# Project-SEA-Stack/HydroChrono

Hardware: AMD Instinct MI355X
Metric: hydro-force evals/sec (all bodies) (higher is better)
Workload: dtype f64

## Files before the change

hydrochrono_amd/csrc/hc_kernels.hpp:

```cpp
#pragma once
#include <hip/hip_runtime.h>

#include <cstddef>

#include "hc_limits.hpp"
#include "hc_tail.hpp"

namespace hc {


struct Panel {
    const double* base;
    int ntiles;
    int ngp;
};
inline size_t panel_doubles(int ntiles, int ngp) { return static_cast<size_t>(ntiles) * ngp * 128; }

struct HistoryView {
    const double* state;
    int N, D;
    double t;
    const double* ring_t;
    const double* ring_v;
    const double* ring_vT;
// ... 245 lines not shown
ScatterLaunch scatter_launch_config(ScatterArgs& a);
FinalizeLaunch finalize_launch_config(FinalizeArgs& a);
struct StepLaunch {
    int nblocks = 0;
    size_t smem = 0;
    int MT = 0;
    static constexpr int U = 2;
};
StepLaunch step_launch_config(const StepArgs& a, int mt);
struct BlockLaunch {
    int nblocks = 0;
    size_t smem = 0;
    int MT = 0, R = 0, NB = 0, WPS = 0;
};
BlockLaunch block_launch_config(const BlockArgs& a, int mt, BlockArgs* with_lds_layout);

void launch_relayout_rirf(const double* d_Kb_6xDxS, double* d_K, int ngp, int D, int S, int row0, double scale, hipStream_t stream);
void launch_relayout_rowmajor(const double* d_src, int rows, int cols, double* d_panel, int ngp, int row0, hipStream_t stream);
void launch_conv_step(const StepArgs& a, int mt, hipStream_t stream);
void launch_conv_block(const BlockArgs& a, int mt, hipStream_t stream);
void launch_reduce_block(const ReduceArgs& r, hipStream_t stream);
int reduce_block_grid(const ReduceArgs& r);
void launch_finalize(const FinalizeArgs& a, hipStream_t stream);
void launch_near_split(const NearArgs& a, hipStream_t stream);
void launch_wide_step(const WideStepArgs& a, hipStream_t stream);
void launch_scatter(const ScatterArgs& a, hipStream_t stream);
void launch_taper(const TaperArgs& a, hipStream_t stream);
void launch_eta_synthesis(const double* d_t, int nt, const double* d_amp, const double* d_omega, const double* d_phase, int nf,
                          double ramp_duration, double* d_eta, hipStream_t stream);
void launch_added_mass_mv(const double* d_M, int rows, int cols, const double* d_w, double c, double* d_R, hipStream_t stream);
void launch_added_mass_mv_tagged(const double* d_M, int rows, int cols, const double* d_w, const double* d_R_in, double c,
                                 unsigned long long* d_tagged, unsigned long long seq, const double* d_canary_in, unsigned long long* d_canary_out,
                                 hipStream_t stream);
void launch_unrelayout(const Panel& K, int Dloc, int D, int S, double* d_out, hipStream_t stream);
void launch_extract_series(const Panel& K, int row, int col, int D, int S, double* d_out, hipStream_t stream);
void launch_ring_transpose(const double* d_ring_v, int Hcap, int HcapT, int D, double* d_ring_vT, hipStream_t stream);
void launch_synth_rirf(double* d_K, int ntiles, int ngp, int Dloc, int D, int S, int row0, double dt, unsigned long long seed, double rho,
                       hipStream_t stream);

struct TailKhatArgs {
    Panel K;
    const double* width;
    const double* tw;
    double* Khat;
    int Dloc, D, S, NP;
};

struct TailFwdArgs {
    const double* ring_vT;
    int HcapT, Hcap, head;
    int D, S, NP;
    const double* tw;
    double* Xw;
};

struct TailGemvArgs {
    const double* Khat;
    const double* Xw;
    const double* Yin;
    double* Yout;
    int Dloc, ncols;
    int bin_lo, bin_hi;
    int col_lo, col_hi;
    int x_shift;
    int rows_per_wg;
};

struct TailInvArgs {
    const double* Y;
    const double* tw;
    double* tail;
    int Dloc, Dpad;
};
constexpr int kTailGemvRows = 32;
int tail_gemv_lds_bytes(const TailGemvArgs& g);
int tail_gemv_grid(const TailGemvArgs& g);
hipError_t launch_tail_khat(const TailKhatArgs& a, int N, hipStream_t s);
hipError_t launch_tail_fwd(const TailFwdArgs& a, int N, hipStream_t s);
void launch_tail_gemv(const TailGemvArgs& a, hipStream_t s);
hipError_t launch_tail_inv(const TailInvArgs& a, int N, hipStream_t s);

}
```

hydrochrono_amd/csrc/hc_pass.cpp:

```cpp
#include "hc_internal.hpp"

using namespace hc::detail;

namespace hc {
namespace detail {

StepViews make_views(const hc_ctx* c) {
    StepViews v{};
    const bool irregular = c->wave_kind == hc::kWaveIrregular;
    v.kex.base   = c->d_kex.p;
    v.kex.ntiles = c->ntiles;
    v.kex.ngp    = c->ngp_ex;
    v.ex.L        = c->L;
    v.ex.ex_tau   = c->d_ex_tau.p;
    v.ex.ex_width = c->d_ex_width.p;
    v.ex.eta_t    = c->d_eta_t.p;
    v.ex.eta      = c->d_eta.p;
    v.ex.nt       = c->nt;
    v.ex.eta_dt   = irregular ? (c->eta_record ? c->eta_h : c->irr.simulation_dt) : 1.0;
    v.ex.eta_t0   = (irregular && !c->eta_t.empty()) ? c->eta_t.front() : 0.0;
    return v;
}


// ... 134 lines not shown
    c->spec.far_cur = c->spec.far_next = 0;
    if (k_changed)
        for (auto& f : c->spec_form) f.khat_ok = false;
}

namespace {

int spec_n_index(int N) { return N == 256 ? 0 : (N == 512 ? 1 : 2); }
int spec_form_index(const hc_ctx* c) { return c->radiation_tail == hc::kTailFormUniform ? 1 : 0; }

bool spec_eligible(const hc_ctx* c, bool direct) {
    const auto& pl = c->plan;
    if (c->radiation_tail != hc::kTailFormLevelled && c->radiation_tail != hc::kTailFormUniform) return false;
    hc::TailLevel lv[hc::kTailLevelsMax];
    const int nlev = hc::tail_levels(c->S, c->radiation_tail, lv);
    if (nlev < 1) return false;
    if (direct) {
        if (!c->dk_tail_gemv.ok()) return false;
        for (int l = 0; l < nlev; ++l)
            if (!c->dk_tail_fwd[spec_n_index(lv[l].N)].ok() || !c->dk_tail_inv[spec_n_index(lv[l].N)].ok()) return false;
    }
    if (c->conv_mode == 1 && !c->proc_ready) return false;
    if (c->pass_ahead == 1 || (c->pass_ahead == 2 && c->ahead_now && pass_ahead_size_ok(c))) return false;
    const int L = c->lookahead;
    const int NP = hc::tail_partitions(c->S);
    if ((L != 16 && L != 32) || c->D >= 1024 || NP < 1 || NP * c->D > hc::kTailMaxCols) return false;
    if (!pl.valid || pl.own_zero || pl.sub != 0) return false;
    const int head = hc::tail_head_lags(lv, nlev);
    for (int j = 0; j < L; ++j)
        if (pl.s_defer[j] >= 0 || pl.s_cut[j] >= head) return false;
    return hc::tail_grid_ok(c->times, c->tau, pl.dt, pl.tgrid[1]);
}

void spec_twiddles(hc_ctx* c, hc_ctx::SpectralLevel& lev) {
    const int N = lev.lv.N;
    if (lev.tw.n == static_cast<size_t>(2 * N)) return;
    std::vector<double> tw(2 * static_cast<size_t>(N));
    const double pi = 3.14159265358979323846;
    for (int k = 0; k < N; ++k) {
        const int q = (4 * k) / N, r = k - q * (N / 4);
        const double cr = std::cos(2.0 * pi * r / N), sr = std::sin(2.0 * pi * r / N);
        double co = cr, si = sr;
        if (q == 1) { co = -sr; si = cr; }
        if (q == 2) { co = -cr; si = -sr; }
        if (q == 3) { co = sr; si = -cr; }
        tw[2 * k]     = co;
        tw[2 * k + 1] = -si;
    }
    lev.tw.alloc(tw.size());
    HC_HIP(hipMemcpyAsync(lev.tw.p, tw.data(), tw.size() * sizeof(double), hipMemcpyHostToDevice, c->stream));
    HC_HIP(hipStreamSynchronize(c->stream));
}

void spec_dispatch_gemv(hc_ctx* c, const hc_ctx::SpectralLevel& lev, hipStream_t stream, bool direct, int bin_lo, int bin_hi, int col_lo, int col_hi, int x_shift,
                        const double* Yin, double* Yout) {
    if (bin_hi <= bin_lo || col_hi <= col_lo) return;
    hc::TailGemvArgs g{};
    g.Khat = lev.khat.p;
    g.Xw   = lev.xw.p;
    g.Yin  = Yin;
    g.Yout = Yout;
    g.Dloc = c->Dloc;
    g.ncols = lev.lv.NP * c->D;
    g.bin_lo = bin_lo;
    g.bin_hi = bin_hi;
    g.col_lo = col_lo;
    g.col_hi = col_hi;
    g.x_shift = x_shift;
    g.rows_per_wg = hc::kTailGemvRows;
    const double bytes = 16.0 * (bin_hi - bin_lo) * (static_cast<double>(c->Dloc) * (col_hi - col_lo) + (col_hi - col_lo) + (Yin ? 2.0 : 1.0) * c->Dloc);
    c->prof.tail_bytes += bytes;
    c->prof.tail_launches += 1;
    if (direct) {
        c->dq->dispatch(c->dk_tail_gemv, static_cast<uint32_t>(hc::tail_gemv_grid(g)), 256, static_cast<uint32_t>(hc::tail_gemv_lds_bytes(g)), &g, sizeof g,
                        direct_tag(c, hc::kEvTail));
        c->prof.direct_dispatches += 1;
        return;
    }
    hc::EventPair* ev = ev_begin(c, hc::kEvTail, stream);
    hc::launch_tail_gemv(g, stream);
    ev_end(ev, stream);
    c->prof.hip_launches += 1;
}

void spec_level_start(hc_ctx* c, hc_ctx::SpectralLevel& lev, bool top, hipStream_t stream, bool direct) {
    auto& sp = c->spec;
    const hc::TailLevel& lv = lev.lv;
    const int NP = lv.NP, D = c->D;
    const bool dd = direct;
    hc::TailFwdArgs f{};
    f.ring_vT = c->d_ring_vT.p;
    f.HcapT   = c->HcapT;
    f.Hcap    = c->Hcap;
    f.head    = c->head;
    f.D       = D;
    f.S       = c->S;
    f.NP      = NP;
    f.tw      = lev.tw.p;
    f.Xw      = lev.xw.p;
    c->prof.tail_bytes += 8.0 * NP * D * lv.N + 16.0 * lv.bins * NP * D;
    c->prof.tail_launches += 1;
    if (dd) {
        c->dq->dispatch(c->dk_tail_fwd[spec_n_index(lv.N)], static_cast<uint32_t>(NP * D), lv.N / 2, 0, &f, sizeof f, direct_tag(c, hc::kEvTail));
        c->prof.direct_dispatches += 1;
    } else {
        hc::EventPair* ev = ev_begin(c, hc::kEvTail, stream);
        HC_HIP(hc::launch_tail_fwd(f, lv.N, stream));
        ev_end(ev, stream);
        c->prof.hip_launches += 1;
    }
    double* Y = lev.y.p + static_cast<size_t>(top ? sp.cur : 0) * 2 * lv.bins * c->Dloc;
    if (NP > 1) {
        const int nch = hc::tail_far_chunks(sp.Q);
        if (!top || !hc::tail_level_far_ahead(lv) || sp.far_cur == 0) {
            spec_dispatch_gemv(c, lev, stream, dd, 0, lv.bins, D, NP * D, hc::tail_x_shift(false, D), nullptr, Y);
        } else {
            for (int k = 0; k < nch; ++k) {
                if (sp.far_cur & (1u << k)) continue;
                int lo, hi;
                hc::tail_level_chunk_bins(lv, k, nch, &lo, &hi);
                spec_dispatch_gemv(c, lev, stream, dd, lo, hi, D, NP * D, hc::tail_x_shift(false, D), nullptr, Y);
            }
        }
    }
    spec_dispatch_gemv(c, lev, stream, dd, 0, lv.bins, 0, D, 0, NP > 1 ? Y : nullptr, Y);
    hc::TailInvArgs iv{Y, lev.tw.p, lev.out.p, c->Dloc, c->Dpad};
    c->prof.tail_bytes += 16.0 * lv.bins * c->Dloc + 8.0 * lv.P * c->Dloc;
    c->prof.tail_launches += 1;
    if (dd) {
        c->dq->dispatch(c->dk_tail_inv[spec_n_index(lv.N)], static_cast<uint32_t>(c->Dloc), lv.N / 2, 0, &iv, sizeof iv, direct_tag(c, hc::kEvTail));
        c->prof.direct_dispatches += 1;
    } else {
        hc::EventPair* ev = ev_begin(c, hc::kEvTail, stream);
        HC_HIP(hc::launch_tail_inv(iv, lv.N, stream));
        ev_end(ev, stream);
        c->prof.hip_launches += 1;
    }
}

bool spec_ready(hc_ctx* c) {
    auto& form = c->spec_form[spec_form_index(c)];
    hc::TailLevel lv[hc::kTailLevelsMax];
    const int nlev = hc::tail_levels(c->S, c->radiation_tail, lv);
    if (nlev < 1) return false;
    if (form.nlev != nlev || form.S != c->S) form.khat_ok = false;
    form.nlev = nlev;
    form.S    = c->S;
    std::vector<hc::DeviceBuffer<double>*> fresh;
    auto grow = [&](hc::DeviceBuffer<double>& b, size_t n) {
        if (b.n >= n) return false;
        fresh.push_back(&b);
        b.alloc(n);
        return true;
    };
    try {
        for (int l = 0; l < nlev; ++l) {
            auto& lev = form.lev[l];
            lev.lv = lv[l];
            const size_t bins = static_cast<size_t>(lv[l].bins), ncols = static_cast<size_t>(lv[l].NP) * c->D;
            grow(lev.xw, 2 * bins * ncols);
            grow(lev.y, 4 * bins * c->Dloc);
            if (grow(lev.out, static_cast<size_t>(lv[l].P) * c->Dpad)) {
                HC_HIP(hipMemsetAsync(lev.out.p, 0, lev.out.n * sizeof(double), c->stream));
                HC_HIP(hipStreamSynchronize(c->stream));
            }
            if (grow(lev.khat, 2 * bins * c->Dloc * ncols)) form.khat_ok = false;
        }
    } catch (const Error&) {
        (void)hipGetLastError();
        for (auto* b : fresh) b->release();
        form.khat_ok      = false;
        c->radiation_tail = 0;
        return false;
    }
    for (int l = 0; l < nlev; ++l) spec_twiddles(c, form.lev[l]);
    if (!form.khat_ok) {
        for (int l = 0; l < nlev; ++l) spec_build_khat(c, form.lev[l]);
        form.khat_ok = true;
    }
    return form.khat_ok;
}

}

void launch_pass(hc_ctx* c, hipStream_t stream, bool with_exc, bool direct, bool spec_goes_on) {
    auto& sp = c->spec;
    const auto& pl = c->plan;
    const int L = c->lookahead;
    const int fi = spec_form_index(c);
    bool use_tail = false;
    if (spec_goes_on && sp.active && sp.form == fi && sp.k < sp.Q && std::fabs(pl.dt - sp.dt) <= 1e-9 * sp.dt) {
        const double tol = std::max(1e-9 * pl.dt, 64.0 * std::numeric_limits<double>::epsilon() * std::fabs(pl.tgrid[1]));
        use_tail = std::fabs(pl.tgrid[1] - (sp.t0 + sp.k * L * sp.dt)) <= tol;
    }
    if (!use_tail) {
        const bool follows = spec_goes_on && sp.active && sp.form == fi && sp.k == sp.Q &&
                             std::fabs(pl.tgrid[1] - (sp.t0 + sp.k * L * sp.dt)) <=
                                 std::max(1e-9 * pl.dt, 64.0 * std::numeric_limits<double>::epsilon() * std::fabs(pl.tgrid[1])) &&
                             std::fabs(pl.dt - sp.dt) <= 1e-9 * sp.dt;
        const unsigned far_made = follows ? sp.far_next : 0u;
        sp.active = false;
        if (spec_eligible(c, direct) && spec_ready(c)) {
            sp.form     = fi;
            sp.cur      = follows ? 1 - sp.cur : sp.cur;
            sp.far_cur  = far_made;
            sp.far_next = 0;
            sp.Q        = hc::tail_level_blocks(c->spec_form[fi].lev[0].lv, L);
            sp.k        = 0;
            sp.t0       = pl.tgrid[1];
            sp.dt       = pl.dt;
            sp.active   = true;
            use_tail = true;
        }
    }
    if (!use_tail) {
        const PassSetup ps = make_pass(c, with_exc, false);
        c->plan.has_exc    = ps.exc_block;
        issue_pass_chunks(c, ps, 0, ps.b.nchunks, true, stream, direct);
        issue_pass_reduce(c, ps, rows_P(c, false), rows_E(c, false), stream, direct);
        return;
    }
    auto& form = c->spec_form[fi];
    const int j0 = sp.k * L;
    TailRows rows;
    for (int l = 0; l < form.nlev; ++l) {
        auto& lev = form.lev[l];
        if (hc::tail_level_starts(lev.lv, j0)) spec_level_start(c, lev, l == 0, stream, direct);
        rows.tail[l] = lev.out.p;
        rows.j0[l]   = j0 % lev.lv.period;
    }
    const PassSetup ps = make_pass(c, with_exc, false, hc::tail_head_lags(&form.lev[form.nlev - 1].lv, 1));
    c->plan.has_exc    = ps.exc_block;
    issue_pass_chunks(c, ps, 0, ps.b.nchunks, true, stream, direct);
    issue_pass_reduce(c, ps, rows_P(c, false), rows_E(c, false), stream, direct, 0, &rows);
    const auto& top = form.lev[0];
    const int NP = top.lv.NP;
    if (hc::tail_level_far_ahead(top.lv) && sp.k >= 1) {
        const int ch = sp.k - 1, nch = hc::tail_far_chunks(sp.Q);
        int lo, hi;
        hc::tail_level_chunk_bins(top.lv, ch, nch, &lo, &hi);
        spec_dispatch_gemv(c, top, stream, direct, lo, hi, c->D, NP * c->D, hc::tail_x_shift(true, c->D), nullptr,
                           top.y.p + static_cast<size_t>(1 - sp.cur) * 2 * top.lv.bins * c->Dloc);
        sp.far_next |= 1u << ch;
    }
    sp.k += 1;
    sp.serial = c->plan_serial;
    c->prof.tail_blocks += 1;
}

void ahead_drop(hc_ctx* c) { c->ahead.active = false; }

void reset_schedule_state(hc_ctx* c) {
    c->gap_seen = c->gap_long = c->gap_long_lo = 0;
    c->gap_hint  = -1.0;
    c->ahead_now = hc::near_slices_for(c->D) > 1 && c->gap_threshold <= 0.0;
}

bool schedule_ahead_for_next_block(hc_ctx* c) {
    if (c->pass_ahead == 0 || c->lookahead > 32) return false;
    if (c->pass_ahead == 1) return true;
    if (!pass_ahead_size_ok(c)) return false;
    if (c->gap_seen >= std::max(4, c->lookahead / 4)) {
        c->ahead_now = 2 * (c->ahead_now ? c->gap_long_lo : c->gap_long) > c->gap_seen;
        c->gap_seen = c->gap_long = c->gap_long_lo = 0;
    }
    (c->ahead_now ? c->prof.schedule_blocks_ahead : c->prof.schedule_blocks_at_start) += 1;
    return c->ahead_now;
}

void ahead_issue_slice(hc_ctx* c, hipStream_t stream, bool direct) {
    auto& ah = c->ahead;
    if (!ah.active || ah.reduced) return;
    if (ah.Hcap != c->Hcap || ah.plan_serial != c->plan_serial) { ahead_drop(c); return; }
    const int pushed = ((c->head - ah.head0) % c->Hcap + c->Hcap) % c->Hcap;
    if (std::max(pushed, c->lookahead) + ah.Hv - 2 >= c->Hcap) { ahead_drop(c); return; }
    PassSetup ps;
    ps.b         = ah.args;
    ps.b.hist.ring_t  = c->d_ring_t.p;
    ps.b.hist.ring_v  = c->d_ring_v.p;
    ps.b.hist.ring_vT = c->d_ring_vT.p;
    ps.exc_block = ah.has_exc;
    ps.rad_once  = ah.rad_once;
// ... 213 lines not shown
```

hydrochrono_amd/csrc/hc_runtime.cpp:

```cpp
#include "hc_internal.hpp"

#include <sched.h>

#include <cctype>

#include <atomic>

using namespace hc::detail;

template <class T>
void hc::BarBuffer<T>::alloc(size_t count) {
    if (p) (void)hipFree(p);
    p       = nullptr;
    n       = 0;
    host_ok = false;
    if (count == 0) return;
    static const bool disabled = HC_TUNE_INT("HC_NO_BAR_STATE", 0) != 0;
    if (disabled) return;
    void* q = nullptr;
    if (hipExtMallocWithFlags(&q, count * sizeof(T), hipDeviceMallocFinegrained) != hipSuccess) {
        (void)hipGetLastError();
        return;
    }
    p = static_cast<T*>(q);
// ... 552 lines not shown
                *abandon      = true;
            }
            return false;
        }
        const unsigned long long bits = tag[0];
        double got;
        std::memcpy(&got, &bits, sizeof got);
        if (got != rv + cv * wv) {
            c->direct_why = "self-test of the direct dispatch: memory re-written through the PCIe BAR was read stale";
            (void)q->drain(2.0, lane);
            return false;
        }
    }
    if (!q->drain(2.0, lane)) {
        c->direct_why = "self-test of the direct dispatch timed out";
        *abandon      = true;
        return false;
    }
    return true;
}

#ifdef HC_TUNING
static const char* const kKernelObjectName = "/hc_kernels_tuning.co";
#else
static const char* const kKernelObjectName = "/hc_kernels.co";
#endif
__attribute__((constructor)) static void request_device_memory_queue_rings() {
    if (env_int("HC_QUEUE_DEV_MEM", 0) == 0) return;
    (void)setenv("HSA_ALLOCATE_QUEUE_DEV_MEM", "1", 0);
}

void setup_direct(hc_ctx* c) {
    c->direct_ready = false;
    if (env_int("HC_DIRECT", 1) == 0) { c->direct_why = "disabled by HC_DIRECT=0"; return; }
    if (!c->bar_state.host_ok || !c->bar_am.host_ok || !c->bar_selftest.host_ok) { c->direct_why = "the device's memory is not host-addressable"; return; }
    std::unique_ptr<hc::DirectQueue> q(new hc::DirectQueue);
    std::string why;
    if (!q->init(c->device, library_dir() + kKernelObjectName, &why)) { c->direct_why = why; return; }
    c->dk_finalize = q->find("finalize_kernelILi4ELb0EEEv");
    c->dk_finalize_slot = q->find("finalize_kernelILi4ELb1EEEv");
    c->dk_scatter  = q->find("scatter_kernelE");
    c->dk_near     = q->find("near_split_kernelE");
    c->dk_wide     = q->find("wide_step_kernelE");
    if (c->dk_wide.kernarg != sizeof(hc::WideStepArgs) || c->dk_wide.priv != 0) c->dk_wide = hc::DirectKernel{};
    if (c->dk_finalize_slot.kernarg != sizeof(hc::FinalizeArgs) || c->dk_finalize_slot.priv != 0) c->dk_finalize_slot = hc::DirectKernel{};
    c->slot_state = HC_TUNE_INT("HC_SLOT_STATE", 1) != 0 && c->dk_finalize_slot.ok() && c->N <= hc::kSlotStateMaxBodies;
    c->dk_step_hot[0] = q->find("step_hot_kernelILi1EEEv");
    c->dk_step_hot[1] = q->find("step_hot_kernelILi2EEEv");
    for (auto& k : c->dk_step_hot)
        if (k.kernarg != sizeof(hc::StepHotArgs) || k.priv != 0) k = hc::DirectKernel{};
    c->step_hot = c->slot_state && c->dk_step_hot[0].ok() && c->dk_step_hot[1].ok() && HC_TUNE_INT("HC_STEP_HOT", 1) != 0;
    c->step_halves = HC_TUNE_INT("HC_STEP_HALVES", 1) == 2 ? 2 : 1;
    c->dk_reduce   = q->find("reduce_block_kernelE");
    c->dk_tail_gemv = q->find("tail_gemvENS_12TailGemvArgsE");
    bool tail_ok    = c->dk_tail_gemv.kernarg == sizeof(hc::TailGemvArgs) && !c->dk_tail_gemv.priv;
    for (int i = 0; i < 3; ++i) {
        char frag[64];
        std::snprintf(frag, sizeof frag, "tail_fft_fwdILi%dEEEvNS_11TailFwdArgsE", 256 << i);
        c->dk_tail_fwd[i] = q->find(frag);
        std::snprintf(frag, sizeof frag, "tail_fft_invILi%dEEEvNS_11TailInvArgsE", 256 << i);
        c->dk_tail_inv[i] = q->find(frag);
        tail_ok = tail_ok && c->dk_tail_fwd[i].kernarg == sizeof(hc::TailFwdArgs) && c->dk_tail_inv[i].kernarg == sizeof(hc::TailInvArgs) && !c->dk_tail_fwd[i].priv &&
                  !c->dk_tail_inv[i].priv;
    }
    if (!tail_ok) {
        c->dk_tail_gemv = hc::DirectKernel{};
        for (int i = 0; i < 3; ++i) c->dk_tail_fwd[i] = c->dk_tail_inv[i] = hc::DirectKernel{};
    }
    c->dk_added_mass = q->find("added_mass_mv_tagged_kernelE");
    {
        hc::StepArgs a{};
        a.ngroups = 1;
        const hc::StepLaunch l = hc::step_launch_config(a, c->mt);
        char frag[64];
        std::snprintf(frag, sizeof frag, "conv_step_kernelILi%dELi%dEEEv", l.MT, hc::StepLaunch::U);
        c->dk_step = q->find(frag);
        if (c->dk_step.kernarg != sizeof(hc::StepArgs) || c->dk_step.priv != 0) c->dk_step = hc::DirectKernel{};
    }
    for (int depth : {16, 32}) {
        hc::BlockArgs a{}, b{};
        a.depth = depth;
        a.ngroups = 1;
        const hc::BlockLaunch l = hc::block_launch_config(a, c->mt_block, &b);
        char frag[96];
        std::snprintf(frag, sizeof frag, "conv_block_kernelILi%dELi%dELi%dELi%dEEEv", l.MT, l.R, l.NB, l.WPS);
        (depth == 16 ? c->dk_block16 : c->dk_block32) = q->find(frag);
        const hc::BlockLaunch lm = hc::block_launch_config(a, c->mt_mini, &b);
        std::snprintf(frag, sizeof frag, "conv_block_kernelILi%dELi%dELi%dELi%dEEEv", lm.MT, lm.R, lm.NB, lm.WPS);
        (depth == 16 ? c->dk_mini16 : c->dk_mini32) = q->find(frag);
        if (depth == 16) {
            const hc::BlockLaunch ln = hc::block_launch_config(a, c->mt_narrow, &b);
            std::snprintf(frag, sizeof frag, "conv_block_kernelILi%dELi%dELi%dELi%dEEEv", ln.MT, ln.R, ln.NB, ln.WPS);
            c->dk_narrow = q->find(frag);
        }
    }
#ifdef HC_TUNING
    {
        hc::BlockArgs a{}, b{};
        a.depth   = 64;
        a.ngroups = 1;
        const hc::BlockLaunch l = hc::block_launch_config(a, hc::kBlock64MT, &b);
        char frag[96];
        std::snprintf(frag, sizeof frag, "conv_block_kernelILi%dELi%dELi%dELi%dEEEv", l.MT, l.R, l.NB, l.WPS);
        c->dk_block64 = q->find(frag);
        if (c->dk_block64.kernarg != sizeof(hc::BlockArgs) || c->dk_block64.priv != 0) c->dk_block64 = hc::DirectKernel{};
    }
#endif
    if (!c->dk_narrow.ok() || c->dk_narrow.priv || c->dk_narrow.kernarg != sizeof(hc::BlockArgs)) {
        c->direct_why = "the narrow short-pass variant of the pass kernel is missing from hc_kernels.co";
        return;
    }
    if (!c->dk_mini16.ok() || !c->dk_mini32.ok() || c->dk_mini16.priv || c->dk_mini32.priv || c->dk_mini16.kernarg != sizeof(hc::BlockArgs) ||
        c->dk_mini32.kernarg != sizeof(hc::BlockArgs)) {
        c->direct_why = "the short-pass variant of the pass kernel is missing from hc_kernels.co";
        return;
// ... 63 lines not shown
```

hydrochrono_amd/csrc/hc_tail_kernels.hpp:

```cpp
#pragma once

namespace hc {

template <int N>
__device__ __forceinline__ void tail_fft_lds(double* __restrict__ re, double* __restrict__ im, const double* __restrict__ tw, bool inverse) {
    const int t = threadIdx.x;
    __syncthreads();
#pragma unroll 1
    for (int len = 2; len <= N; len <<= 1) {
        const int half = len >> 1;
        const int pos  = t & (half - 1);
        const int i    = (t - pos) * 2 + pos;
        const int j    = i + half;
        const int k    = pos * (N / len);
        const double wr = tw[2 * k], wi = inverse ? -tw[2 * k + 1] : tw[2 * k + 1];
        const double br = re[j], bi = im[j];
        const double pr = wr * br - wi * bi, pi = wr * bi + wi * br;
        const double ar = re[i], ai = im[i];
        re[i] = ar + pr;
        im[i] = ai + pi;
        re[j] = ar - pr;
        im[j] = ai - pi;
        __syncthreads();
    }
}

constexpr int tail_log2(int n) { return n <= 1 ? 0 : 1 + tail_log2(n >> 1); }
template <int N>
__device__ __forceinline__ int tail_bitrev(int k) {
    static_assert(N >= 4 && (N & (N - 1)) == 0, "a transform of 2^b points");
    return static_cast<int>(__brev(static_cast<unsigned>(k)) >> (32 - tail_log2(N)));
}


template <int N>
__global__ void __launch_bounds__(N / 2) tail_khat_kernel(TailKhatArgs a) {
    constexpr int P = N / 2, kBins = P + 1, kThreads = N / 2;
    __shared__ double re[N], im[N];
    const int t   = threadIdx.x;
    const int col = blockIdx.x % a.D;
    const int rp  = blockIdx.x / a.D;
    const int p   = rp % a.NP + 1;
    const int row = rp / a.NP;
    for (int k = t; k < N; k += kThreads) {
        const int s = p * P + k;
        double g = 0.0;
        if (k < P && s < a.S) g = a.width[s] * a.K.base[panel_offset(a.K.ngp, row, s * a.D + col)];
        const int kr = tail_bitrev<N>(k);
        re[kr] = g;
        im[kr] = 0.0;
    }
    tail_fft_lds<N>(re, im, a.tw, false);
    const size_t ncols = static_cast<size_t>(a.NP) * a.D;
    const size_t c     = static_cast<size_t>(p - 1) * a.D + col;
    for (int b = t; b < kBins; b += kThreads) {
        double* dst = a.Khat + 2 * ((static_cast<size_t>(b) * a.Dloc + row) * ncols + c);
        dst[0] = re[b];
        dst[1] = im[b];
    }
}


template <int N>
__global__ void __launch_bounds__(N / 2) tail_fft_fwd(TailFwdArgs a) {
    constexpr int P = N / 2, kBins = P + 1, kThreads = N / 2;
    __shared__ double re[N], im[N];
    const int t   = threadIdx.x;
    const int col = blockIdx.x % a.D;
    const int w   = blockIdx.x / a.D + 1;
    const double* __restrict__ series = a.ring_vT + static_cast<size_t>(col) * a.HcapT;
    for (int k = t; k < N; k += kThreads) {
        const int back = (w + 1) * P - 1 - k;
        double x = 0.0;
        if (k >= 1 && back <= a.S - 2) {
            int slot = (a.head - back) % a.Hcap;
            if (slot < 0) slot += a.Hcap;
            x = series[slot];
        }
        const int kr = tail_bitrev<N>(k);
        re[kr] = x;
        im[kr] = 0.0;
    }
    tail_fft_lds<N>(re, im, a.tw, false);
    const size_t ncols = static_cast<size_t>(a.NP) * a.D;
    const size_t c     = static_cast<size_t>(w - 1) * a.D + col;
    for (int b = t; b < kBins; b += kThreads) {
        double* dst = a.Xw + 2 * (static_cast<size_t>(b) * ncols + c);
        dst[0] = re[b];
        dst[1] = im[b];
    }
}

static constexpr int kTailGemvUnroll = 6;
static constexpr int kTailGemvBatch  = 4;

__global__ void __launch_bounds__(256) tail_gemv(TailGemvArgs a) {
    extern __shared__ double xs[];
    const int nbin_rows = (a.Dloc + a.rows_per_wg - 1) / a.rows_per_wg;
    const int bin       = a.bin_lo + blockIdx.x / nbin_rows;
    const int row0      = (blockIdx.x % nbin_rows) * a.rows_per_wg;
    const int n         = a.col_hi - a.col_lo;
    const double* __restrict__ xsrc = a.Xw + 2 * (static_cast<size_t>(bin) * a.ncols + a.col_lo + a.x_shift);
    for (int i = threadIdx.x; i < 2 * n; i += 256) xs[i] = xsrc[i];
    __syncthreads();
    const int lane = threadIdx.x & 63, wave = threadIdx.x >> 6;
    const int row_end = min(a.Dloc, row0 + a.rows_per_wg);
    const dvec2* __restrict__ kbin = reinterpret_cast<const dvec2*>(a.Khat + 2 * (static_cast<size_t>(bin) * a.Dloc * a.ncols + a.col_lo));
    for (int rb = row0 + wave * kTailGemvBatch; rb < row_end; rb += 4 * kTailGemvBatch) {
        double sr[kTailGemvBatch], si[kTailGemvBatch];
#pragma unroll
        for (int q = 0; q < kTailGemvBatch; ++q) sr[q] = si[q] = 0.0;
        for (int c0 = 0; c0 < n; c0 += 64 * kTailGemvUnroll) {
            dvec2 kv[kTailGemvBatch][kTailGemvUnroll];
#pragma unroll
            for (int q = 0; q < kTailGemvBatch; ++q) {
                const int row = min(rb + q, row_end - 1);
#pragma unroll
                for (int u = 0; u < kTailGemvUnroll; ++u) {
                    const int c = c0 + 64 * u + lane;
                    kv[q][u] = c < n ? __builtin_nontemporal_load(kbin + static_cast<size_t>(row) * a.ncols + c) : dvec2{0.0, 0.0};
                }
            }
#pragma unroll
            for (int u = 0; u < kTailGemvUnroll; ++u) {
                const int c = c0 + 64 * u + lane;
                const double xr = c < n ? xs[2 * c] : 0.0, xi = c < n ? xs[2 * c + 1] : 0.0;
#pragma unroll
                for (int q = 0; q < kTailGemvBatch; ++q) {
                    sr[q] = fma(kv[q][u].x, xr, sr[q]);
                    sr[q] = fma(-kv[q][u].y, xi, sr[q]);
                    si[q] = fma(kv[q][u].x, xi, si[q]);
                    si[q] = fma(kv[q][u].y, xr, si[q]);
                }
            }
        }
#pragma unroll
        for (int off = 32; off >= 1; off >>= 1) {
#pragma unroll
            for (int q = 0; q < kTailGemvBatch; ++q) {
                sr[q] += __shfl_xor(sr[q], off, 64);
                si[q] += __shfl_xor(si[q], off, 64);
            }
        }
        if (lane < kTailGemvBatch && rb + lane < row_end) {
            double yr = sr[0], yi = si[0];
#pragma unroll
            for (int q = 1; q < kTailGemvBatch; ++q)
                if (lane == q) {
                    yr = sr[q];
                    yi = si[q];
                }
            const size_t o = 2 * (static_cast<size_t>(bin) * a.Dloc + rb + lane);
            if (a.Yin) {
                yr = a.Yin[o] + yr;
                yi = a.Yin[o + 1] + yi;
            }
            a.Yout[o]     = yr;
            a.Yout[o + 1] = yi;
        }
    }
}

template <int N>
__global__ void __launch_bounds__(N / 2) tail_fft_inv(TailInvArgs a) {
    constexpr int P = N / 2, kThreads = N / 2;
    __shared__ double re[N], im[N];
    const int t   = threadIdx.x;
    const int row = blockIdx.x;
    for (int k = t; k < N; k += kThreads) {
        const int b = k <= P ? k : N - k;
        const double* y = a.Y + 2 * (static_cast<size_t>(b) * a.Dloc + row);
        const double yr = y[0];
        double yi       = (b == 0 || b == P) ? 0.0 : y[1];
        if (k > P) yi = -yi;
        const int kr = tail_bitrev<N>(k);
        re[kr] = yr;
        im[kr] = yi;
    }
    tail_fft_lds<N>(re, im, a.tw, true);
    for (int j = t; j < P; j += kThreads) a.tail[static_cast<size_t>(j) * a.Dpad + row] = re[P + j] * (1.0 / N);
}

int tail_gemv_lds_bytes(const TailGemvArgs& g) { return 16 * (g.col_hi - g.col_lo); }
int tail_gemv_grid(const TailGemvArgs& g) { return (g.bin_hi - g.bin_lo) * ((g.Dloc + g.rows_per_wg - 1) / g.rows_per_wg); }

template __global__ void tail_khat_kernel<256>(TailKhatArgs);
template __global__ void tail_khat_kernel<512>(TailKhatArgs);
template __global__ void tail_khat_kernel<1024>(TailKhatArgs);
template __global__ void tail_fft_fwd<256>(TailFwdArgs);
template __global__ void tail_fft_fwd<512>(TailFwdArgs);
template __global__ void tail_fft_fwd<1024>(TailFwdArgs);
template __global__ void tail_fft_inv<256>(TailInvArgs);
template __global__ void tail_fft_inv<512>(TailInvArgs);
template __global__ void tail_fft_inv<1024>(TailInvArgs);

#define HC_TAIL_BY_N(n, call)                                 \
    switch (n) {                                              \
        case 256: { constexpr int kN = 256; call; break; }    \
        case 512: { constexpr int kN = 512; call; break; }    \
        case 1024: { constexpr int kN = 1024; call; break; }  \
        default: return hipErrorInvalidValue;                 \
    }                                                         \
    return hipSuccess;

hipError_t launch_tail_khat(const TailKhatArgs& a, int N, hipStream_t s) {
    HC_TAIL_BY_N(N, hipLaunchKernelGGL(tail_khat_kernel<kN>, dim3(static_cast<unsigned>(a.Dloc) * a.NP * a.D), dim3(kN / 2), 0, s, a))
}
hipError_t launch_tail_fwd(const TailFwdArgs& a, int N, hipStream_t s) {
    HC_TAIL_BY_N(N, hipLaunchKernelGGL(tail_fft_fwd<kN>, dim3(static_cast<unsigned>(a.NP) * a.D), dim3(kN / 2), 0, s, a))
}
void launch_tail_gemv(const TailGemvArgs& a, hipStream_t s) {
    hipLaunchKernelGGL(tail_gemv, dim3(static_cast<unsigned>(tail_gemv_grid(a))), dim3(256), static_cast<unsigned>(tail_gemv_lds_bytes(a)), s, a);
}
hipError_t launch_tail_inv(const TailInvArgs& a, int N, hipStream_t s) {
    HC_TAIL_BY_N(N, hipLaunchKernelGGL(tail_fft_inv<kN>, dim3(static_cast<unsigned>(a.Dloc)), dim3(kN / 2), 0, s, a))
}
#undef HC_TAIL_BY_N

}
```

Before: 83070.

## Batch spectral tail levels that start together into grouped FFT/GEMV launches

```diff
diff --git a/hydrochrono_amd/csrc/hc_kernels.hpp b/hydrochrono_amd/csrc/hc_kernels.hpp
--- a/hydrochrono_amd/csrc/hc_kernels.hpp
+++ b/hydrochrono_amd/csrc/hc_kernels.hpp
@@ -321,6 +321,7 @@
     int D, S, NP;
     const double* tw;
     double* Xw;
+    int N;
 };
 
 struct TailGemvArgs {
@@ -340,13 +341,26 @@
     const double* tw;
     double* tail;
     int Dloc, Dpad;
-};
+    int N;
+};
+
+template <class Args>
+struct TailGroup {
+    Args lev[kTailLevelsMax];
+    int wg_end[kTailLevelsMax];
+};
+using TailFwdGroup  = TailGroup<TailFwdArgs>;
+using TailGemvGroup = TailGroup<TailGemvArgs>;
+using TailInvGroup  = TailGroup<TailInvArgs>;
+
 constexpr int kTailGemvRows = 32;
 int tail_gemv_lds_bytes(const TailGemvArgs& g);
 int tail_gemv_grid(const TailGemvArgs& g);
+inline int tail_fwd_grid(const TailFwdArgs& a) { return a.NP * a.D; }
+inline int tail_inv_grid(const TailInvArgs& a) { return a.Dloc; }
 hipError_t launch_tail_khat(const TailKhatArgs& a, int N, hipStream_t s);
-hipError_t launch_tail_fwd(const TailFwdArgs& a, int N, hipStream_t s);
-void launch_tail_gemv(const TailGemvArgs& a, hipStream_t s);
-hipError_t launch_tail_inv(const TailInvArgs& a, int N, hipStream_t s);
+hipError_t launch_tail_fwd(const TailFwdGroup& g, int workgroups, hipStream_t s);
+void launch_tail_gemv(const TailGemvGroup& g, int workgroups, int lds_bytes, hipStream_t s);
+hipError_t launch_tail_inv(const TailInvGroup& g, int workgroups, hipStream_t s);
 
 }
diff --git a/hydrochrono_amd/csrc/hc_pass.cpp b/hydrochrono_amd/csrc/hc_pass.cpp
--- a/hydrochrono_amd/csrc/hc_pass.cpp
+++ b/hydrochrono_amd/csrc/hc_pass.cpp
@@ -210,9 +210,8 @@
     HC_HIP(hipStreamSynchronize(c->stream));
 }
 
-void spec_dispatch_gemv(hc_ctx* c, const hc_ctx::SpectralLevel& lev, hipStream_t stream, bool direct, int bin_lo, int bin_hi, int col_lo, int col_hi, int x_shift,
-                        const double* Yin, double* Yout) {
-    if (bin_hi <= bin_lo || col_hi <= col_lo) return;
+hc::TailGemvArgs spec_gemv_args(const hc_ctx* c, const hc_ctx::SpectralLevel& lev, int bin_lo, int bin_hi, int col_lo, int col_hi, int x_shift, const double* Yin,
+                                double* Yout) {
     hc::TailGemvArgs g{};
     g.Khat = lev.khat.p;
     g.Xw   = lev.xw.p;
@@ -226,71 +225,112 @@
     g.col_hi = col_hi;
     g.x_shift = x_shift;
     g.rows_per_wg = hc::kTailGemvRows;
-    const double bytes = 16.0 * (bin_hi - bin_lo) * (static_cast<double>(c->Dloc) * (col_hi - col_lo) + (col_hi - col_lo) + (Yin ? 2.0 : 1.0) * c->Dloc);
-    c->prof.tail_bytes += bytes;
+    return g;
+}
+
+template <class Args, class GridOf>
+int spec_group_ends(hc::TailGroup<Args>& g, int n, GridOf grid_of) {
+    int end = 0;
+    for (int l = 0; l < hc::kTailLevelsMax; ++l) {
+        if (l < n) end += grid_of(g.lev[l]);
+        else g.lev[l] = g.lev[n - 1];
+        g.wg_end[l] = end;
+    }
+    return end;
+}
+
+void spec_dispatch_gemv(hc_ctx* c, hc::TailGemvGroup& g, int n, hipStream_t stream, bool direct) {
+    int lds = 0;
+    for (int l = 0; l < n; ++l) {
+        const hc::TailGemvArgs& a = g.lev[l];
+        lds = std::max(lds, hc::tail_gemv_lds_bytes(a));
+        c->prof.tail_bytes += 16.0 * (a.bin_hi - a.bin_lo) *
+                              (static_cast<double>(c->Dloc) * (a.col_hi - a.col_lo) + (a.col_hi - a.col_lo) + (a.Yin ? 2.0 : 1.0) * c->Dloc);
+    }
+    const int wgs = spec_group_ends(g, n, [](const hc::TailGemvArgs& a) { return hc::tail_gemv_grid(a); });
     c->prof.tail_launches += 1;
     if (direct) {
-        c->dq->dispatch(c->dk_tail_gemv, static_cast<uint32_t>(hc::tail_gemv_grid(g)), 256, static_cast<uint32_t>(hc::tail_gemv_lds_bytes(g)), &g, sizeof g,
-                        direct_tag(c, hc::kEvTail));
+        c->dq->dispatch(c->dk_tail_gemv, static_cast<uint32_t>(wgs), 256, static_cast<uint32_t>(lds), &g, sizeof g, direct_tag(c, hc::kEvTail));
         c->prof.direct_dispatches += 1;
         return;
     }
     hc::EventPair* ev = ev_begin(c, hc::kEvTail, stream);
-    hc::launch_tail_gemv(g, stream);
+    hc::launch_tail_gemv(g, wgs, lds, stream);
     ev_end(ev, stream);
     c->prof.hip_launches += 1;
 }
 
-void spec_level_start(hc_ctx* c, hc_ctx::SpectralLevel& lev, bool top, hipStream_t stream, bool direct) {
+void spec_dispatch_gemv(hc_ctx* c, const hc_ctx::SpectralLevel& lev, hipStream_t stream, bool direct, int bin_lo, int bin_hi, int col_lo, int col_hi, int x_shift,
+                        const double* Yin, double* Yout) {
+    if (bin_hi <= bin_lo || col_hi <= col_lo) return;
+    hc::TailGemvGroup g{};
+    g.lev[0] = spec_gemv_args(c, lev, bin_lo, bin_hi, col_lo, col_hi, x_shift, Yin, Yout);
+    spec_dispatch_gemv(c, g, 1, stream, direct);
+}
+
+void spec_levels_start(hc_ctx* c, hc_ctx::SpectralLevel* const* lev, int n, bool top, hipStream_t stream, bool direct) {
     auto& sp = c->spec;
-    const hc::TailLevel& lv = lev.lv;
-    const int NP = lv.NP, D = c->D;
-    const bool dd = direct;
-    hc::TailFwdArgs f{};
-    f.ring_vT = c->d_ring_vT.p;
-    f.HcapT   = c->HcapT;
-    f.Hcap    = c->Hcap;
-    f.head    = c->head;
-    f.D       = D;
-    f.S       = c->S;
-    f.NP      = NP;
-    f.tw      = lev.tw.p;
-    f.Xw      = lev.xw.p;
-    c->prof.tail_bytes += 8.0 * NP * D * lv.N + 16.0 * lv.bins * NP * D;
+    const int D = c->D;
+    hc::TailFwdGroup fg{};
+    hc::TailGemvGroup ng{};
+    hc::TailInvGroup ig{};
+    double* Y[hc::kTailLevelsMax];
+    for (int l = 0; l < n; ++l) {
+        const hc::TailLevel& lv = lev[l]->lv;
+        hc::TailFwdArgs& f = fg.lev[l];
+        f.ring_vT = c->d_ring_vT.p;
+        f.HcapT   = c->HcapT;
+        f.Hcap    = c->Hcap;
+        f.head    = c->head;
+        f.D       = D;
+        f.S       = c->S;
+        f.NP      = lv.NP;
+        f.tw      = lev[l]->tw.p;
+        f.Xw      = lev[l]->xw.p;
+        f.N       = lv.N;
+        c->prof.tail_bytes += 8.0 * lv.NP * D * lv.N + 16.0 * lv.bins * lv.NP * D;
+        Y[l] = lev[l]->y.p + static_cast<size_t>(top && l == 0 ? sp.cur : 0) * 2 * lv.bins * c->Dloc;
+    }
+    const int fwd_wgs = spec_group_ends(fg, n, [](const hc::TailFwdArgs& a) { return hc::tail_fwd_grid(a); });
     c->prof.tail_launches += 1;
-    if (dd) {
-        c->dq->dispatch(c->dk_tail_fwd[spec_n_index(lv.N)], static_cast<uint32_t>(NP * D), lv.N / 2, 0, &f, sizeof f, direct_tag(c, hc::kEvTail));
+    if (direct) {
+        c->dq->dispatch(c->dk_tail_fwd[spec_n_index(fg.lev[0].N)], static_cast<uint32_t>(fwd_wgs), fg.lev[0].N / 2, 0, &fg, sizeof fg, direct_tag(c, hc::kEvTail));
         c->prof.direct_dispatches += 1;
     } else {
         hc::EventPair* ev = ev_begin(c, hc::kEvTail, stream);
-        HC_HIP(hc::launch_tail_fwd(f, lv.N, stream));
+        HC_HIP(hc::launch_tail_fwd(fg, fwd_wgs, stream));
         ev_end(ev, stream);
         c->prof.hip_launches += 1;
     }
-    double* Y = lev.y.p + static_cast<size_t>(top ? sp.cur : 0) * 2 * lv.bins * c->Dloc;
-    if (NP > 1) {
-        const int nch = hc::tail_far_chunks(sp.Q);
-        if (!top || !hc::tail_level_far_ahead(lv) || sp.far_cur == 0) {
-            spec_dispatch_gemv(c, lev, stream, dd, 0, lv.bins, D, NP * D, hc::tail_x_shift(false, D), nullptr, Y);
-        } else {
-            for (int k = 0; k < nch; ++k) {
-                if (sp.far_cur & (1u << k)) continue;
-                int lo, hi;
-                hc::tail_level_chunk_bins(lv, k, nch, &lo, &hi);
-                spec_dispatch_gemv(c, lev, stream, dd, lo, hi, D, NP * D, hc::tail_x_shift(false, D), nullptr, Y);
+    for (int l = 0; l < n; ++l) {
+        const hc::TailLevel& lv = lev[l]->lv;
+        const int NP = lv.NP;
+        if (NP > 1) {
+            const int nch = hc::tail_far_chunks(sp.Q);
+            if (!(top && l == 0) || !hc::tail_level_far_ahead(lv) || sp.far_cur == 0) {
+                spec_dispatch_gemv(c, *lev[l], stream, direct, 0, lv.bins, D, NP * D, hc::tail_x_shift(false, D), nullptr, Y[l]);
+            } else {
+                for (int k = 0; k < nch; ++k) {
+                    if (sp.far_cur & (1u << k)) continue;
+                    int lo, hi;
+                    hc::tail_level_chunk_bins(lv, k, nch, &lo, &hi);
+                    spec_dispatch_gemv(c, *lev[l], stream, direct, lo, hi, D, NP * D, hc::tail_x_shift(false, D), nullptr, Y[l]);
+                }
             }
         }
-    }
-    spec_dispatch_gemv(c, lev, stream, dd, 0, lv.bins, 0, D, 0, NP > 1 ? Y : nullptr, Y);
-    hc::TailInvArgs iv{Y, lev.tw.p, lev.out.p, c->Dloc, c->Dpad};
-    c->prof.tail_bytes += 16.0 * lv.bins * c->Dloc + 8.0 * lv.P * c->Dloc;
+        ng.lev[l] = spec_gemv_args(c, *lev[l], 0, lv.bins, 0, D, 0, NP > 1 ? Y[l] : nullptr, Y[l]);
+        ig.lev[l] = hc::TailInvArgs{Y[l], lev[l]->tw.p, lev[l]->out.p, c->Dloc, c->Dpad, lv.N};
+        c->prof.tail_bytes += 16.0 * lv.bins * c->Dloc + 8.0 * lv.P * c->Dloc;
+    }
+    spec_dispatch_gemv(c, ng, n, stream, direct);
+    const int inv_wgs = spec_group_ends(ig, n, [](const hc::TailInvArgs& a) { return hc::tail_inv_grid(a); });
     c->prof.tail_launches += 1;
-    if (dd) {
-        c->dq->dispatch(c->dk_tail_inv[spec_n_index(lv.N)], static_cast<uint32_t>(c->Dloc), lv.N / 2, 0, &iv, sizeof iv, direct_tag(c, hc::kEvTail));
+    if (direct) {
+        c->dq->dispatch(c->dk_tail_inv[spec_n_index(ig.lev[0].N)], static_cast<uint32_t>(inv_wgs), ig.lev[0].N / 2, 0, &ig, sizeof ig, direct_tag(c, hc::kEvTail));
         c->prof.direct_dispatches += 1;
     } else {
         hc::EventPair* ev = ev_begin(c, hc::kEvTail, stream);
-        HC_HIP(hc::launch_tail_inv(iv, lv.N, stream));
+        HC_HIP(hc::launch_tail_inv(ig, inv_wgs, stream));
         ev_end(ev, stream);
         c->prof.hip_launches += 1;
     }
@@ -381,11 +421,18 @@
     auto& form = c->spec_form[fi];
     const int j0 = sp.k * L;
     TailRows rows;
+    hc_ctx::SpectralLevel* starting[hc::kTailLevelsMax];
+    int nstart = 0;
     for (int l = 0; l < form.nlev; ++l) {
         auto& lev = form.lev[l];
-        if (hc::tail_level_starts(lev.lv, j0)) spec_level_start(c, lev, l == 0, stream, direct);
+        if (hc::tail_level_starts(lev.lv, j0)) starting[nstart++] = &lev;
         rows.tail[l] = lev.out.p;
         rows.j0[l]   = j0 % lev.lv.period;
+    }
+    if (HC_TUNE_INT("HC_TAIL_GROUP", 1) != 0) {
+        if (nstart > 0) spec_levels_start(c, starting, nstart, j0 == 0, stream, direct);
+    } else {
+        for (int i = 0; i < nstart; ++i) spec_levels_start(c, starting + i, 1, j0 == 0 && i == 0, stream, direct);
     }
     const PassSetup ps = make_pass(c, with_exc, false, hc::tail_head_lags(&form.lev[form.nlev - 1].lv, 1));
     c->plan.has_exc    = ps.exc_block;
diff --git a/hydrochrono_amd/csrc/hc_runtime.cpp b/hydrochrono_amd/csrc/hc_runtime.cpp
--- a/hydrochrono_amd/csrc/hc_runtime.cpp
+++ b/hydrochrono_amd/csrc/hc_runtime.cpp
@@ -628,15 +628,15 @@
     c->step_hot = c->slot_state && c->dk_step_hot[0].ok() && c->dk_step_hot[1].ok() && HC_TUNE_INT("HC_STEP_HOT", 1) != 0;
     c->step_halves = HC_TUNE_INT("HC_STEP_HALVES", 1) == 2 ? 2 : 1;
     c->dk_reduce   = q->find("reduce_block_kernelE");
-    c->dk_tail_gemv = q->find("tail_gemvENS_12TailGemvArgsE");
-    bool tail_ok    = c->dk_tail_gemv.kernarg == sizeof(hc::TailGemvArgs) && !c->dk_tail_gemv.priv;
+    c->dk_tail_gemv = q->find("tail_gemvENS_9TailGroupINS_12TailGemvArgsEEE");
+    bool tail_ok    = c->dk_tail_gemv.kernarg == sizeof(hc::TailGemvGroup) && !c->dk_tail_gemv.priv;
     for (int i = 0; i < 3; ++i) {
-        char frag[64];
-        std::snprintf(frag, sizeof frag, "tail_fft_fwdILi%dEEEvNS_11TailFwdArgsE", 256 << i);
+        char frag[96];
+        std::snprintf(frag, sizeof frag, "tail_fft_fwdILi%dEEEvNS_9TailGroupINS_11TailFwdArgsEEE", 256 << i);
         c->dk_tail_fwd[i] = q->find(frag);
-        std::snprintf(frag, sizeof frag, "tail_fft_invILi%dEEEvNS_11TailInvArgsE", 256 << i);
+        std::snprintf(frag, sizeof frag, "tail_fft_invILi%dEEEvNS_9TailGroupINS_11TailInvArgsEEE", 256 << i);
         c->dk_tail_inv[i] = q->find(frag);
-        tail_ok = tail_ok && c->dk_tail_fwd[i].kernarg == sizeof(hc::TailFwdArgs) && c->dk_tail_inv[i].kernarg == sizeof(hc::TailInvArgs) && !c->dk_tail_fwd[i].priv &&
+        tail_ok = tail_ok && c->dk_tail_fwd[i].kernarg == sizeof(hc::TailFwdGroup) && c->dk_tail_inv[i].kernarg == sizeof(hc::TailInvGroup) && !c->dk_tail_fwd[i].priv &&
                   !c->dk_tail_inv[i].priv;
     }
     if (!tail_ok) {
diff --git a/hydrochrono_amd/csrc/hc_tail_kernels.hpp b/hydrochrono_amd/csrc/hc_tail_kernels.hpp
--- a/hydrochrono_amd/csrc/hc_tail_kernels.hpp
+++ b/hydrochrono_amd/csrc/hc_tail_kernels.hpp
@@ -8,22 +8,46 @@
     __syncthreads();
 #pragma unroll 1
     for (int len = 2; len <= N; len <<= 1) {
-        const int half = len >> 1;
-        const int pos  = t & (half - 1);
-        const int i    = (t - pos) * 2 + pos;
-        const int j    = i + half;
-        const int k    = pos * (N / len);
-        const double wr = tw[2 * k], wi = inverse ? -tw[2 * k + 1] : tw[2 * k + 1];
-        const double br = re[j], bi = im[j];
-        const double pr = wr * br - wi * bi, pi = wr * bi + wi * br;
-        const double ar = re[i], ai = im[i];
-        re[i] = ar + pr;
-        im[i] = ai + pi;
-        re[j] = ar - pr;
-        im[j] = ai - pi;
+        if (t < N / 2) {
+            const int half = len >> 1;
+            const int pos  = t & (half - 1);
+            const int i    = (t - pos) * 2 + pos;
+            const int j    = i + half;
+            const int k    = pos * (N / len);
+            const double wr = tw[2 * k], wi = inverse ? -tw[2 * k + 1] : tw[2 * k + 1];
+            const double br = re[j], bi = im[j];
+            const double pr = wr * br - wi * bi, pi = wr * bi + wi * br;
+            const double ar = re[i], ai = im[i];
+            re[i] = ar + pr;
+            im[i] = ai + pi;
+            re[j] = ar - pr;
+            im[j] = ai - pi;
+        }
         __syncthreads();
     }
 }
+
+template <class Args>
+__device__ __forceinline__ Args tail_group_level(const TailGroup<Args>& g, int* wg) {
+    static_assert(kTailLevelsMax == 3, "the selection below is written out for three levels");
+    const int b = static_cast<int>(blockIdx.x);
+    Args a = g.lev[0];
+    *wg    = b;
+    if (b >= g.wg_end[0]) {
+        a   = g.lev[1];
+        *wg = b - g.wg_end[0];
+    }
+    if (b >= g.wg_end[1]) {
+        a   = g.lev[2];
+        *wg = b - g.wg_end[1];
+    }
+    return a;
+}
+
+#define HC_TAIL_BODY_BY_N(NMAX, n, call)                                                   \
+    if (NMAX >= 1024 && (n) == 1024) { constexpr int kN = NMAX >= 1024 ? 1024 : NMAX; call; } \
+    else if (NMAX >= 512 && (n) == 512) { constexpr int kN = NMAX >= 512 ? 512 : NMAX; call; } \
+    else { constexpr int kN = 256; call; }
 
 constexpr int tail_log2(int n) { return n <= 1 ? 0 : 1 + tail_log2(n >> 1); }
 template <int N>
@@ -62,43 +86,54 @@
 
 
 template <int N>
-__global__ void __launch_bounds__(N / 2) tail_fft_fwd(TailFwdArgs a) {
+__device__ __forceinline__ void tail_fwd_level(const TailFwdArgs& a, int wg, double* __restrict__ re, double* __restrict__ im) {
     constexpr int P = N / 2, kBins = P + 1, kThreads = N / 2;
-    __shared__ double re[N], im[N];
     const int t   = threadIdx.x;
-    const int col = blockIdx.x % a.D;
-    const int w   = blockIdx.x / a.D + 1;
+    const int col = wg % a.D;
+    const int w   = wg / a.D + 1;
     const double* __restrict__ series = a.ring_vT + static_cast<size_t>(col) * a.HcapT;
-    for (int k = t; k < N; k += kThreads) {
-        const int back = (w + 1) * P - 1 - k;
-        double x = 0.0;
-        if (k >= 1 && back <= a.S - 2) {
-            int slot = (a.head - back) % a.Hcap;
-            if (slot < 0) slot += a.Hcap;
-            x = series[slot];
-        }
-        const int kr = tail_bitrev<N>(k);
-        re[kr] = x;
-        im[kr] = 0.0;
-    }
+    if (t < kThreads)
+        for (int k = t; k < N; k += kThreads) {
+            const int back = (w + 1) * P - 1 - k;
+            double x = 0.0;
+            if (k >= 1 && back <= a.S - 2) {
+                int slot = (a.head - back) % a.Hcap;
+                if (slot < 0) slot += a.Hcap;
+                x = series[slot];
+            }
+            const int kr = tail_bitrev<N>(k);
+            re[kr] = x;
+            im[kr] = 0.0;
+        }
     tail_fft_lds<N>(re, im, a.tw, false);
     const size_t ncols = static_cast<size_t>(a.NP) * a.D;
     const size_t c     = static_cast<size_t>(w - 1) * a.D + col;
-    for (int b = t; b < kBins; b += kThreads) {
-        double* dst = a.Xw + 2 * (static_cast<size_t>(b) * ncols + c);
-        dst[0] = re[b];
-        dst[1] = im[b];
-    }
+    if (t < kThreads)
+        for (int b = t; b < kBins; b += kThreads) {
+            double* dst = a.Xw + 2 * (static_cast<size_t>(b) * ncols + c);
+            dst[0] = re[b];
+            dst[1] = im[b];
+        }
+}
+
+template <int NMAX>
+__global__ void __launch_bounds__(NMAX / 2) tail_fft_fwd(TailFwdGroup g) {
+    __shared__ double re[NMAX], im[NMAX];
+    int wg;
+    const TailFwdArgs a = tail_group_level(g, &wg);
+    HC_TAIL_BODY_BY_N(NMAX, a.N, tail_fwd_level<kN>(a, wg, re, im))
 }
 
 static constexpr int kTailGemvUnroll = 6;
 static constexpr int kTailGemvBatch  = 4;
 
-__global__ void __launch_bounds__(256) tail_gemv(TailGemvArgs a) {
+__global__ void __launch_bounds__(256) tail_gemv(TailGemvGroup g) {
     extern __shared__ double xs[];
+    int wg;
+    const TailGemvArgs a = tail_group_level(g, &wg);
     const int nbin_rows = (a.Dloc + a.rows_per_wg - 1) / a.rows_per_wg;
-    const int bin       = a.bin_lo + blockIdx.x / nbin_rows;
-    const int row0      = (blockIdx.x % nbin_rows) * a.rows_per_wg;
+    const int bin       = a.bin_lo + wg / nbin_rows;
+    const int row0      = (wg % nbin_rows) * a.rows_per_wg;
     const int n         = a.col_hi - a.col_lo;
     const double* __restrict__ xsrc = a.Xw + 2 * (static_cast<size_t>(bin) * a.ncols + a.col_lo + a.x_shift);
     for (int i = threadIdx.x; i < 2 * n; i += 256) xs[i] = xsrc[i];
@@ -162,24 +197,33 @@
 }
 
 template <int N>
-__global__ void __launch_bounds__(N / 2) tail_fft_inv(TailInvArgs a) {
+__device__ __forceinline__ void tail_inv_level(const TailInvArgs& a, int row, double* __restrict__ re, double* __restrict__ im) {
     constexpr int P = N / 2, kThreads = N / 2;
-    __shared__ double re[N], im[N];
-    const int t   = threadIdx.x;
-    const int row = blockIdx.x;
-    for (int k = t; k < N; k += kThreads) {
-        const int b = k <= P ? k : N - k;
-        const double* y = a.Y + 2 * (static_cast<size_t>(b) * a.Dloc + row);
-        const double yr = y[0];
-        double yi       = (b == 0 || b == P) ? 0.0 : y[1];
-        if (k > P) yi = -yi;
-        const int kr = tail_bitrev<N>(k);
-        re[kr] = yr;
-        im[kr] = yi;
-    }
+    const int t = threadIdx.x;
+    if (t < kThreads)
+        for (int k = t; k < N; k += kThreads) {
+            const int b = k <= P ? k : N - k;
+            const double* y = a.Y + 2 * (static_cast<size_t>(b) * a.Dloc + row);
+            const double yr = y[0];
+            double yi       = (b == 0 || b == P) ? 0.0 : y[1];
+            if (k > P) yi = -yi;
+            const int kr = tail_bitrev<N>(k);
+            re[kr] = yr;
+            im[kr] = yi;
+        }
     tail_fft_lds<N>(re, im, a.tw, true);
-    for (int j = t; j < P; j += kThreads) a.tail[static_cast<size_t>(j) * a.Dpad + row] = re[P + j] * (1.0 / N);
-}
+    if (t < kThreads)
+        for (int j = t; j < P; j += kThreads) a.tail[static_cast<size_t>(j) * a.Dpad + row] = re[P + j] * (1.0 / N);
+}
+
+template <int NMAX>
+__global__ void __launch_bounds__(NMAX / 2) tail_fft_inv(TailInvGroup g) {
+    __shared__ double re[NMAX], im[NMAX];
+    int row;
+    const TailInvArgs a = tail_group_level(g, &row);
+    HC_TAIL_BODY_BY_N(NMAX, a.N, tail_inv_level<kN>(a, row, re, im))
+}
+#undef HC_TAIL_BODY_BY_N
 
 int tail_gemv_lds_bytes(const TailGemvArgs& g) { return 16 * (g.col_hi - g.col_lo); }
 int tail_gemv_grid(const TailGemvArgs& g) { return (g.bin_hi - g.bin_lo) * ((g.Dloc + g.rows_per_wg - 1) / g.rows_per_wg); }
@@ -187,12 +231,12 @@
 template __global__ void tail_khat_kernel<256>(TailKhatArgs);
 template __global__ void tail_khat_kernel<512>(TailKhatArgs);
 template __global__ void tail_khat_kernel<1024>(TailKhatArgs);
-template __global__ void tail_fft_fwd<256>(TailFwdArgs);
-template __global__ void tail_fft_fwd<512>(TailFwdArgs);
-template __global__ void tail_fft_fwd<1024>(TailFwdArgs);
-template __global__ void tail_fft_inv<256>(TailInvArgs);
-template __global__ void tail_fft_inv<512>(TailInvArgs);
-template __global__ void tail_fft_inv<1024>(TailInvArgs);
+template __global__ void tail_fft_fwd<256>(TailFwdGroup);
+template __global__ void tail_fft_fwd<512>(TailFwdGroup);
+template __global__ void tail_fft_fwd<1024>(TailFwdGroup);
+template __global__ void tail_fft_inv<256>(TailInvGroup);
+template __global__ void tail_fft_inv<512>(TailInvGroup);
+template __global__ void tail_fft_inv<1024>(TailInvGroup);
 
 #define HC_TAIL_BY_N(n, call)                                 \
     switch (n) {                                              \
@@ -206,14 +250,14 @@
 hipError_t launch_tail_khat(const TailKhatArgs& a, int N, hipStream_t s) {
     HC_TAIL_BY_N(N, hipLaunchKernelGGL(tail_khat_kernel<kN>, dim3(static_cast<unsigned>(a.Dloc) * a.NP * a.D), dim3(kN / 2), 0, s, a))
 }
-hipError_t launch_tail_fwd(const TailFwdArgs& a, int N, hipStream_t s) {
-    HC_TAIL_BY_N(N, hipLaunchKernelGGL(tail_fft_fwd<kN>, dim3(static_cast<unsigned>(a.NP) * a.D), dim3(kN / 2), 0, s, a))
-}
-void launch_tail_gemv(const TailGemvArgs& a, hipStream_t s) {
-    hipLaunchKernelGGL(tail_gemv, dim3(static_cast<unsigned>(tail_gemv_grid(a))), dim3(256), static_cast<unsigned>(tail_gemv_lds_bytes(a)), s, a);
-}
-hipError_t launch_tail_inv(const TailInvArgs& a, int N, hipStream_t s) {
-    HC_TAIL_BY_N(N, hipLaunchKernelGGL(tail_fft_inv<kN>, dim3(static_cast<unsigned>(a.Dloc)), dim3(kN / 2), 0, s, a))
+hipError_t launch_tail_fwd(const TailFwdGroup& g, int workgroups, hipStream_t s) {
+    HC_TAIL_BY_N(g.lev[0].N, hipLaunchKernelGGL(tail_fft_fwd<kN>, dim3(static_cast<unsigned>(workgroups)), dim3(kN / 2), 0, s, g))
+}
+void launch_tail_gemv(const TailGemvGroup& g, int workgroups, int lds_bytes, hipStream_t s) {
+    hipLaunchKernelGGL(tail_gemv, dim3(static_cast<unsigned>(workgroups)), dim3(256), static_cast<unsigned>(lds_bytes), s, g);
+}
+hipError_t launch_tail_inv(const TailInvGroup& g, int workgroups, hipStream_t s) {
+    HC_TAIL_BY_N(g.lev[0].N, hipLaunchKernelGGL(tail_fft_inv<kN>, dim3(static_cast<unsigned>(workgroups)), dim3(kN / 2), 0, s, g))
 }
 #undef HC_TAIL_BY_N
 
diff --git a/profiles/tail_fixed/trace_split.py b/profiles/tail_fixed/trace_split.py
--- /dev/null
+++ b/profiles/tail_fixed/trace_split.py
@@ -0,0 +1,66 @@
+import csv
+import re
+import sys
+from collections import defaultdict
+
+TAIL = ("tail_fft_fwd", "tail_gemv", "tail_fft_inv", "conv_block_kernel", "reduce_block_kernel")
+
+
+def short(name):
+    return re.sub(r"\(.*", "", name).replace("void ", "")
+
+
+def main(path, label):
+    rows = []
+    with open(path) as f:
+        for r in csv.DictReader(f):
+            rows.append((int(r["Start_Timestamp"]), int(r["End_Timestamp"]), short(r["Kernel_Name"]),
+                         int(r["Grid_Size_X"]) // max(1, int(r["Workgroup_Size_X"]))))
+    rows.sort()
+    is_tail = lambda n: any(t in n for t in TAIL)
+    stats = defaultdict(list)
+    for b, e, n, wgs in rows:
+        if is_tail(n):
+            stats[(n, wgs)].append(e - b)
+    print(f"## {label}")
+    print(f"{'kernel':<44}{'wgs':>7}{'calls':>7}{'avg_ns':>10}{'min_ns':>10}{'max_ns':>10}{'total_us':>11}")
+    total = 0.0
+    for (n, wgs), d in sorted(stats.items(), key=lambda kv: -sum(kv[1])):
+        if n.startswith("hc::reduce_block_kernel") and len(d) < 4:
+            continue
+        total += sum(d)
+        print(f"{n:<44}{wgs:>7}{len(d):>7}{sum(d) / len(d):>10.0f}{min(d):>10}{max(d):>10}{sum(d) / 1e3:>11.1f}")
+    runs, cur = [], []
+    for r in rows:
+        if is_tail(r[2]):
+            cur.append(r)
+        elif cur:
+            runs.append(cur)
+            cur = []
+    if cur:
+        runs.append(cur)
+    runs = [r for r in runs if any("conv_block_kernel" in x[2] for x in r)]
+    nblocks = len(runs)
+    print(f"pass-and-tail kernel time: {total / 1e3:.1f} us over {nblocks} blocks = {total / 1e3 / nblocks * 16:.0f} us per 16 blocks (512 steps at depth 32)")
+    by_n = defaultdict(list)
+    for r in runs:
+        kern = sum(e - b for b, e, _, _ in r)
+        span = r[-1][1] - r[0][0]
+        gaps = [r[i + 1][0] - r[i][1] for i in range(len(r) - 1)]
+        by_n[len(r)].append((kern, span, gaps))
+    print(f"{'launches in front of the step':<32}{'blocks':>7}{'kernel_us':>11}{'span_us':>10}{'gap mean_us':>13}{'gap min':>9}{'gap max':>9}")
+    all_gaps = []
+    for n, v in sorted(by_n.items()):
+        g = [x for _, _, gs in v for x in gs]
+        all_gaps += g
+        print(f"{n:<32}{len(v):>7}{sum(k for k, _, _ in v) / len(v) / 1e3:>11.1f}{sum(s for _, s, _ in v) / len(v) / 1e3:>10.1f}"
+              f"{sum(g) / max(1, len(g)) / 1e3:>13.2f}{min(g) / 1e3:>9.2f}{max(g) / 1e3:>9.2f}")
+    all_gaps.sort()
+    print(f"gaps between dependent launches at a block start: {len(all_gaps)} gaps, mean {sum(all_gaps) / len(all_gaps) / 1e3:.2f} us, "
+          f"median {all_gaps[len(all_gaps) // 2] / 1e3:.2f} us")
+    spans = sum(s for v in by_n.values() for _, s, _ in v)
+    print(f"span of the block starts (first begin to last end): {spans / 1e3 / nblocks * 16:.0f} us per 16 blocks")
+
+
+if __name__ == "__main__":
+    main(sys.argv[1], sys.argv[2] if len(sys.argv) > 2 else sys.argv[1])
```

New measurement: 83910 (median of 6 runs). No clear change (+1.0%).
